# treangenlab/komb

Measured on NVIDIA B200. Metric: hot-path hits/s (graph build + k-core peel + CORE-A), with peel edges/s and build hits/s, higher is better.
Workload: dtype u32/u64 ids, f64 scores

## Files before the change

komb_b200/csrc/sort.cu:

```cuda
#include "kombgpu_debug.h"
#include "primitives.cuh"

namespace kg {

namespace {

constexpr int kRsThreads = 512;
constexpr int kRsItems = 8;
constexpr int kRsTile = kRsThreads * kRsItems;
constexpr int kRadix = 256;
constexpr int kMaxPasses = 8;

struct DigitSpec {
    int shift, shift2, bits1;
    uint32_t mask1, mask2, mask;
    __host__ __device__ static DigitSpec of(const RadixPass &p) {
        DigitSpec d;
        d.shift = p.shift; d.shift2 = p.shift2; d.bits1 = p.bits;
        d.mask1 = (1u << p.bits) - 1u; d.mask2 = (1u << p.bits2) - 1u;
        d.mask = (1u << (p.bits + p.bits2)) - 1u;
        return d;
    }
    __device__ __forceinline__ uint32_t operator()(uint64_t key) const {
        return ((uint32_t)(key >> shift) & mask1) | (((uint32_t)(key >> shift2) & mask2) << bits1);
    }
};


template <typename W>
struct StatusWord {
    static constexpr int kShift = 8 * (int)sizeof(W) - 2;
    static constexpr W kAgg = W(1) << kShift, kPrefix = W(2) << kShift, kValueMask = (W(1) << kShift) - 1;
    static __device__ __forceinline__ W load(const W *p) {
        W w;
        if constexpr (sizeof(W) == 4) asm volatile("ld.volatile.global.u32 %0, [%1];" : "=r"(w) : "l"(p) : "memory");
        else asm volatile("ld.volatile.global.u64 %0, [%1];" : "=l"(w) : "l"(p) : "memory");
        return w;
    }
    static __device__ __forceinline__ void store(W *p, W w) {
        if constexpr (sizeof(W) == 4) asm volatile("st.volatile.global.u32 [%0], %1;" ::"l"(p), "r"(w) : "memory");
        else asm volatile("st.volatile.global.u64 [%0], %1;" ::"l"(p), "l"(w) : "memory");
    }
};

struct PassList {
    DigitSpec dg[kMaxPasses];
    int n;
};

__global__ void __launch_bounds__(kRsThreads) radix_global_hist_kernel(const uint64_t *__restrict__ keys, uint64_t n, PassList pl,
                                                                       uint32_t *__restrict__ hist) {
    __shared__ uint32_t s_hist[kMaxPasses * kRadix];
    for (int i = threadIdx.x; i < pl.n * kRadix; i += kRsThreads) s_hist[i] = 0;
    __syncthreads();
    const uint32_t lane = lane_id();
    for (uint64_t base = (uint64_t)blockIdx.x * kRsTile; base < n; base += (uint64_t)gridDim.x * kRsTile) {
        uint64_t key[kRsItems];
#pragma unroll
        for (int j = 0; j < kRsItems; ++j) {
            const uint64_t i = base + (uint64_t)j * kRsThreads + threadIdx.x;
            key[j] = i < n ? keys[i] : ~0ull;
        }
#pragma unroll
        for (int j = 0; j < kRsItems; ++j) {
            const uint64_t i = base + (uint64_t)j * kRsThreads + threadIdx.x;
            const bool valid = i < n;
            const bool full = __all_sync(kFullMask, valid);
            for (int p = 0; p < pl.n; ++p) {
                const uint32_t d = pl.dg[p](key[j]);
                const uint32_t d0 = __shfl_sync(kFullMask, d, 0);
                if (full && __all_sync(kFullMask, d == d0)) {
                    if (lane == 0) atomicAdd(&s_hist[p * kRadix + d0], 32u);
                } else if (valid) {
                    atomicAdd(&s_hist[p * kRadix + d], 1u);
                }
            }
        }
    }
    __syncthreads();
    for (int i = threadIdx.x; i < pl.n * kRadix; i += kRsThreads)
        if (s_hist[i]) atomicAdd(&hist[i], s_hist[i]);
}

__global__ void __launch_bounds__(kRadix) radix_hist_scan_kernel(uint32_t *hist) {
    __shared__ uint32_t s_tmp[kRadix / 32 + 1];
    uint32_t *h = hist + (size_t)blockIdx.x * kRadix;
    const uint32_t v = h[threadIdx.x];
    uint32_t total = 0;
    const uint32_t ex = block_excl_scan_add<uint32_t, kRadix>(v, s_tmp, &total);
    h[threadIdx.x] = ex;
}

constexpr int kSweepThreads = 512, kSweepItems = 16, kSweepTile = kSweepThreads * kSweepItems, kSweepMinBlocks = 2;

struct SweepSmem {
    uint64_t keys[kSweepTile];
    uint32_t warp_cnt[kSweepThreads / 32][kRadix];
    uint32_t digit_local[kRadix];
    uint32_t digit_global[kRadix];
    uint32_t digit_total[kRadix];
    uint32_t tile;
};

template <typename W, int kBits>
__global__ void __launch_bounds__(kSweepThreads, kSweepMinBlocks) radix_sweep_kernel(const uint64_t *__restrict__ in, uint64_t *__restrict__ out,
                                                                    uint64_t n, DigitSpec dg,
                                                                    const uint32_t *__restrict__ digit_base,
                                                                    W *status, uint32_t *tile_counter) {
    using SW = StatusWord<W>;
    constexpr int kWarps = kSweepThreads / 32;
    extern __shared__ __align__(16) unsigned char s_raw[];
    SweepSmem &s = *reinterpret_cast<SweepSmem *>(s_raw);
    const uint32_t warp = threadIdx.x >> 5, lane = lane_id();
    const uint32_t mask = kBits ? (1u << kBits) - 1u : dg.mask;
    if (threadIdx.x == 0) s.tile = atomicAdd(tile_counter, 1u);
    for (int i = threadIdx.x; i < kWarps * kRadix; i += kSweepThreads) (&s.warp_cnt[0][0])[i] = 0;
    __syncthreads();
    const uint32_t tile = s.tile;
    const uint64_t tile_base = (uint64_t)tile * kSweepTile;
    const uint32_t tile_count = (uint32_t)min((uint64_t)kSweepTile, n - tile_base);

    uint64_t key[kSweepItems];
    uint16_t rank[kSweepItems];
    const uint32_t warp_base = warp * (32 * kSweepItems);
#pragma unroll
    for (int j = 0; j < kSweepItems; ++j) {
        const uint32_t e = warp_base + j * 32 + lane;
        key[j] = e < tile_count ? in[tile_base + e] : 0;
    }
#pragma unroll
    for (int j = 0; j < kSweepItems; ++j) {
        const uint32_t e = warp_base + j * 32 + lane;
        const bool valid = e < tile_count;
        const uint32_t d = valid ? dg(key[j]) : 0u;
        uint32_t same = __ballot_sync(kFullMask, valid);
#pragma unroll
        for (int b = 0; b < 8; ++b) {
            if (kBits ? (b >= kBits) : ((mask >> b) == 0)) break;
            const uint32_t bit = (d >> b) & 1u;
            const uint32_t vote = __ballot_sync(kFullMask, bit);
            same &= vote ^ (bit - 1u);
        }
        const uint32_t lead = valid ? (uint32_t)__ffs(same) - 1u : lane;
        uint32_t base = 0;
        if (valid && lead == lane) base = atomicAdd(&s.warp_cnt[warp][d], (uint32_t)__popc(same));
        rank[j] = (uint16_t)(__popc(same & lanemask_lt()) + __shfl_sync(kFullMask, base, lead));
    }
    __syncthreads();

    for (uint32_t d = threadIdx.x; d < (uint32_t)kRadix; d += kSweepThreads) {
        uint32_t total = 0;
#pragma unroll
        for (int w = 0; w < kWarps; ++w) {
            const uint32_t c = s.warp_cnt[w][d];
            s.warp_cnt[w][d] = total;
            total += c;
        }
        s.digit_total[d] = total;
        if (d <= mask) SW::store(status + (size_t)tile * kRadix + d, (tile == 0 ? SW::kPrefix : SW::kAgg) | (W)total);
    }
    __syncthreads();
    if (warp == 0) {
        uint32_t v[kRadix / 32], sum = 0;
#pragma unroll
        for (int i = 0; i < kRadix / 32; ++i) { v[i] = s.digit_total[lane * (kRadix / 32) + i]; sum += v[i]; }
        uint32_t run = warp_incl_scan_add(sum) - sum;
#pragma unroll
        for (int i = 0; i < kRadix / 32; ++i) { s.digit_local[lane * (kRadix / 32) + i] = run; run += v[i]; }
    }
    __syncthreads();

#pragma unroll
    for (int j = 0; j < kSweepItems; ++j) {
        const uint32_t e = warp_base + j * 32 + lane;
        if (e < tile_count) {
            const uint32_t d = dg(key[j]);
            s.keys[s.digit_local[d] + s.warp_cnt[warp][d] + rank[j]] = key[j];
        }
    }
    for (uint32_t d = threadIdx.x; d <= mask; d += kSweepThreads) {
        uint32_t excl = 0;
        if (tile > 0) {
            uint32_t p = tile - 1;
            uint32_t spins = 0;
            while (true) {
                const W w = SW::load(status + (size_t)p * kRadix + d);
                if ((w >> SW::kShift) == 0) {
                    if (++spins > (1u << 28)) __trap();
                    continue;
                }
                excl += (uint32_t)(w & SW::kValueMask);
                if (w & SW::kPrefix) break;
                --p;
            }
            SW::store(status + (size_t)tile * kRadix + d, SW::kPrefix | (W)(excl + s.digit_total[d]));
        }
        s.digit_global[d] = digit_base[d] + excl - s.digit_local[d];
    }
    __syncthreads();

    for (uint32_t i = threadIdx.x; i < tile_count; i += kSweepThreads) {
        const uint64_t k = s.keys[i];
        const uint32_t d = dg(k);
        out[(uint64_t)(s.digit_global[d] + i)] = k;
    }
}

template <typename W>
int sweep_pass(kombgpu_ctx *ctx, const uint64_t *src, uint64_t *dst, uint64_t n, const RadixPass &pass, const DigitSpec &dg,
               const uint32_t *digit_base, W *status, uint32_t *tile_counter) {
    auto *kernel = pass.bits + pass.bits2 == 8 ? radix_sweep_kernel<W, 8> : radix_sweep_kernel<W, 0>;
    KG_LAUNCH(ctx, kernel, ceil_div_u64(n, kSweepTile), kSweepThreads, sizeof(SweepSmem), src, dst, n, dg, digit_base, status,
              tile_counter);
    return KOMBGPU_OK;
}

}

int plan_radix_passes(int lo0, int hi0, int lo1, int hi1, RadixPass *out) {
    const int len0 = hi0 > lo0 ? hi0 - lo0 : 0, len1 = hi1 > lo1 ? hi1 - lo1 : 0;
    const int total = len0 + len1;
    if (total <= 0) return 0;
    const int np = (total + 7) / 8;
    const int w = (total + np - 1) / np;
    int n = 0;
    for (int v = 0; v < total; v += w) {
        const int e = v + w < total ? v + w : total;
        RadixPass p{0, 0, 0, 0};
        if (e <= len0) { p.shift = lo0 + v; p.bits = e - v; }
        else if (v >= len0) { p.shift = lo1 + (v - len0); p.bits = e - v; }
        else { p.shift = lo0 + v; p.bits = len0 - v; p.shift2 = lo1; p.bits2 = e - len0; }
        out[n++] = p;
    }
    return n;
}

int radix_sort_u64(kombgpu_ctx *ctx, uint64_t *a, uint64_t *b, uint64_t n, const RadixPass *passes, int n_passes,
                   uint64_t **sorted) {
    *sorted = a;
    if (n < 2 || n_passes == 0) return KOMBGPU_OK;
    if (n >= (1ull << 32)) return ctx_fail(ctx, KOMBGPU_EINVAL, "radix_sort_u64: %llu keys exceed the 2^32 per-array limit", (unsigned long long)n);
    if (n_passes > kMaxPasses) return ctx_fail(ctx, KOMBGPU_EINVAL, "radix_sort_u64: %d passes exceed %d", n_passes, kMaxPasses);
    if (!ctx->sort_attr_set) {
        KG_CUDA(ctx, cudaFuncSetAttribute(radix_sweep_kernel<uint32_t, 8>, cudaFuncAttributeMaxDynamicSharedMemorySize, (int)sizeof(SweepSmem)));
        KG_CUDA(ctx, cudaFuncSetAttribute(radix_sweep_kernel<uint32_t, 0>, cudaFuncAttributeMaxDynamicSharedMemorySize, (int)sizeof(SweepSmem)));
        KG_CUDA(ctx, cudaFuncSetAttribute(radix_sweep_kernel<uint64_t, 8>, cudaFuncAttributeMaxDynamicSharedMemorySize, (int)sizeof(SweepSmem)));
        KG_CUDA(ctx, cudaFuncSetAttribute(radix_sweep_kernel<uint64_t, 0>, cudaFuncAttributeMaxDynamicSharedMemorySize, (int)sizeof(SweepSmem)));
        ctx->sort_attr_set = true;
    }
    const bool wide = n >= (1ull << 30);
    const size_t region = (size_t)ceil_div_u64(n, kSweepTile) * kRadix;
    const size_t head = (size_t)n_passes * kRadix + kMaxPasses;
    const size_t words = head + (wide ? 2 * region : (size_t)n_passes * region);
    DevBuf<uint32_t> ws;
    KG_ALLOC(ctx, ws, words);
    KG_CUDA(ctx, cudaMemsetAsync(ws.p, 0, words * sizeof(uint32_t), ctx->stream));
    PassList pl{};
    pl.n = n_passes;
    for (int p = 0; p < n_passes; ++p) pl.dg[p] = DigitSpec::of(passes[p]);
    uint64_t *src = a, *dst = b;
    const uint32_t hist_grid = min(ceil_div_u64(n, kRsTile), (uint32_t)ctx->sm_count * 4u);
    KG_LAUNCH(ctx, radix_global_hist_kernel, hist_grid, kRsThreads, 0, src, n, pl, ws.p);
    KG_LAUNCH(ctx, radix_hist_scan_kernel, n_passes, kRadix, 0, ws.p);
    for (int p = 0; p < n_passes; ++p) {
        const uint32_t *digit_base = ws.p + (size_t)p * kRadix;
        uint32_t *counter = ws.p + (size_t)n_passes * kRadix + p;
        if (wide) {
            uint64_t *status = reinterpret_cast<uint64_t *>(ws.p + head);
            if (p > 0) KG_CUDA(ctx, cudaMemsetAsync(status, 0, region * sizeof(uint64_t), ctx->stream));
            KG_TRY(sweep_pass(ctx, src, dst, n, passes[p], pl.dg[p], digit_base, status, counter));
        } else {
            KG_TRY(sweep_pass(ctx, src, dst, n, passes[p], pl.dg[p], digit_base, ws.p + head + (size_t)p * region, counter));
        }
        uint64_t *t = src; src = dst; dst = t;
    }
    *sorted = src;
    return KOMBGPU_OK;
}


namespace {

__device__ __forceinline__ uint64_t mix64(uint64_t x) {
    x ^= x >> 33; x *= 0xff51afd7ed558ccdull; x ^= x >> 33; x *= 0xc4ceb9fe1a85ec53ull; x ^= x >> 33;
    return x;
}
__global__ void debug_fill_kernel(uint64_t *keys, uint64_t n, uint64_t lo_mask, uint64_t hi_mask, int sorted_hi) {
    for (uint64_t i = (uint64_t)blockIdx.x * blockDim.x + threadIdx.x; i < n; i += (uint64_t)gridDim.x * blockDim.x) {
        const uint64_t h = mix64(i + 0x9e3779b97f4a7c15ull);
        const uint64_t hi = sorted_hi ? ((i * (hi_mask + 1)) / n) : ((h >> 32) & hi_mask);
        keys[i] = (hi << 32) | (h & lo_mask);
    }
}
__global__ void debug_check_kernel(const uint64_t *keys, uint64_t n, unsigned long long *out) {
    unsigned long long sum = 0, x = 0, bad = 0;
    for (uint64_t i = (uint64_t)blockIdx.x * blockDim.x + threadIdx.x; i < n; i += (uint64_t)gridDim.x * blockDim.x) {
        sum += keys[i];
        x ^= mix64(keys[i]);
        if (i && keys[i - 1] > keys[i]) ++bad;
    }
    atomicAdd(&out[0], sum);
    atomicXor(&out[1], x);
    if (bad) atomicAdd(&out[2], bad);
}

}

}

extern "C" int kombgpu_debug_sort_u64(kombgpu_ctx *ctx, uint64_t n, int lo_bits, int hi_bits, int sorted_hi, int reps,
                                      float *ms_best, int *ok) {
    using namespace kg;
    if (!ctx || !ms_best || !ok || n == 0 || lo_bits < 0 || lo_bits > 32 || hi_bits < 0 || hi_bits > 32 || reps < 1)
        return KOMBGPU_EINVAL;
    KG_CUDA(ctx, cudaSetDevice(ctx->device));
    DevBuf<uint64_t> src, a, b;
    DevBuf<unsigned long long> chk;
    KG_ALLOC(ctx, src, n);
    KG_ALLOC(ctx, a, n);
    KG_ALLOC(ctx, b, n);
    KG_ALLOC(ctx, chk, 6);
    KG_CUDA(ctx, cudaMemsetAsync(chk.p, 0, 6 * sizeof(unsigned long long), ctx->stream));
    const uint64_t lo_mask = lo_bits == 32 ? 0xffffffffull : ((1ull << lo_bits) - 1), hi_mask = hi_bits == 32 ? 0xffffffffull : ((1ull << hi_bits) - 1);
    const int grid = ctx->sm_count * 8;
    KG_LAUNCH(ctx, debug_fill_kernel, grid, 256, 0, src.p, n, lo_mask, hi_mask, sorted_hi);
    KG_LAUNCH(ctx, debug_check_kernel, grid, 256, 0, src.p, n, chk.p);
    RadixPass passes[8];
    const int np = plan_radix_passes(0, lo_bits, 32, 32 + hi_bits, passes);
    float best = 1e30f;
    uint64_t *sorted = nullptr;
    cudaEvent_t e0, e1;
    KG_CUDA(ctx, cudaEventCreate(&e0));
    KG_CUDA(ctx, cudaEventCreate(&e1));
    for (int r = 0; r < reps; ++r) {
        KG_CUDA(ctx, cudaMemcpyAsync(a.p, src.p, n * sizeof(uint64_t), cudaMemcpyDeviceToDevice, ctx->stream));
        KG_CUDA(ctx, cudaEventRecord(e0, ctx->stream));
        int rc = radix_sort_u64(ctx, a.p, b.p, n, passes, np, &sorted);
        if (rc != KOMBGPU_OK) return rc;
        KG_CUDA(ctx, cudaEventRecord(e1, ctx->stream));
        KG_CUDA(ctx, cudaEventSynchronize(e1));
        float ms = 0;
        KG_CUDA(ctx, cudaEventElapsedTime(&ms, e0, e1));
        if (ms < best) best = ms;
    }
    cudaEventDestroy(e0);
    cudaEventDestroy(e1);
    KG_LAUNCH(ctx, debug_check_kernel, grid, 256, 0, sorted, n, chk.p + 3);
    unsigned long long h[6];
    KG_TRY(read_back(ctx, chk.p, h, 6));
    *ok = (h[0] == h[3] && h[1] == h[4] && h[5] == 0) ? 1 : 0;
    *ms_best = best;
    return KOMBGPU_OK;
}
```

Measured before the change: 2.840 billion.

## Widen onesweep radix digits to 10 bits with shared-memory match ranking

Raises the radix from 8 to 10 bits per pass so fewer sweep passes are needed per sort. Warp ranking moves from per-bit ballots to a shared-memory atomicOr match table, with a fast path for warps where all lanes share one digit. Per-warp counts become 16-bit and are handled as digit pairs, and status words are read and written with vector loads and stores. The status buffer is reused across passes with a per-pass memset, and keys are re-read from global memory in the scatter phase to save registers. Risks include bigger shared memory per block lowering occupancy, more decoupled-lookback traffic per tile, and shared-memory atomic contention.

```diff
diff --git a/komb_b200/csrc/sort.cu b/komb_b200/csrc/sort.cu
--- a/komb_b200/csrc/sort.cu
+++ b/komb_b200/csrc/sort.cu
@@ -8,7 +8,8 @@
 constexpr int kRsThreads = 512;
 constexpr int kRsItems = 8;
 constexpr int kRsTile = kRsThreads * kRsItems;
-constexpr int kRadix = 256;
+constexpr int kRadixBits = 10;
+constexpr int kRadix = 1 << kRadixBits;
 constexpr int kMaxPasses = 8;
 
 struct DigitSpec {
@@ -31,15 +32,13 @@
 struct StatusWord {
     static constexpr int kShift = 8 * (int)sizeof(W) - 2;
     static constexpr W kAgg = W(1) << kShift, kPrefix = W(2) << kShift, kValueMask = (W(1) << kShift) - 1;
-    static __device__ __forceinline__ W load(const W *p) {
-        W w;
-        if constexpr (sizeof(W) == 4) asm volatile("ld.volatile.global.u32 %0, [%1];" : "=r"(w) : "l"(p) : "memory");
-        else asm volatile("ld.volatile.global.u64 %0, [%1];" : "=l"(w) : "l"(p) : "memory");
-        return w;
-    }
-    static __device__ __forceinline__ void store(W *p, W w) {
-        if constexpr (sizeof(W) == 4) asm volatile("st.volatile.global.u32 [%0], %1;" ::"l"(p), "r"(w) : "memory");
-        else asm volatile("st.volatile.global.u64 [%0], %1;" ::"l"(p), "l"(w) : "memory");
+    static __device__ __forceinline__ void load2(const W *p, W &a, W &b) {
+        if constexpr (sizeof(W) == 4) asm volatile("ld.volatile.global.v2.u32 {%0, %1}, [%2];" : "=r"(a), "=r"(b) : "l"(p) : "memory");
+        else asm volatile("ld.volatile.global.v2.u64 {%0, %1}, [%2];" : "=l"(a), "=l"(b) : "l"(p) : "memory");
+    }
+    static __device__ __forceinline__ void store2(W *p, W a, W b) {
+        if constexpr (sizeof(W) == 4) asm volatile("st.volatile.global.v2.u32 [%0], {%1, %2};" ::"l"(p), "r"(a), "r"(b) : "memory");
+        else asm volatile("st.volatile.global.v2.u64 [%0], {%1, %2};" ::"l"(p), "l"(a), "l"(b) : "memory");
     }
 };
 
@@ -92,81 +91,98 @@
 }
 
 constexpr int kSweepThreads = 512, kSweepItems = 16, kSweepTile = kSweepThreads * kSweepItems, kSweepMinBlocks = 2;
+constexpr int kSweepWarps = kSweepThreads / 32;
+static_assert(kRadix == 2 * kSweepThreads, "the per-digit phases give every thread the digit pair 2t, 2t+1");
 
 struct SweepSmem {
-    uint64_t keys[kSweepTile];
-    uint32_t warp_cnt[kSweepThreads / 32][kRadix];
+    union {
+        uint64_t keys[kSweepTile];
+        uint32_t match[kSweepWarps][kRadix];
+    };
+    uint16_t warp_cnt[kSweepWarps][kRadix];
     uint32_t digit_local[kRadix];
     uint32_t digit_global[kRadix];
-    uint32_t digit_total[kRadix];
+    uint32_t pair_total[kSweepThreads];
+    uint32_t scan_tmp[kSweepWarps + 1];
     uint32_t tile;
 };
-
-template <typename W, int kBits>
+static_assert(kSweepTile <= 65535, "warp_cnt holds tile positions in 16 bits");
+
+template <typename W>
 __global__ void __launch_bounds__(kSweepThreads, kSweepMinBlocks) radix_sweep_kernel(const uint64_t *__restrict__ in, uint64_t *__restrict__ out,
                                                                     uint64_t n, DigitSpec dg,
                                                                     const uint32_t *__restrict__ digit_base,
                                                                     W *status, uint32_t *tile_counter) {
     using SW = StatusWord<W>;
-    constexpr int kWarps = kSweepThreads / 32;
     extern __shared__ __align__(16) unsigned char s_raw[];
     SweepSmem &s = *reinterpret_cast<SweepSmem *>(s_raw);
     const uint32_t warp = threadIdx.x >> 5, lane = lane_id();
-    const uint32_t mask = kBits ? (1u << kBits) - 1u : dg.mask;
+    const uint32_t mask = dg.mask, radix = mask + 1u;
     if (threadIdx.x == 0) s.tile = atomicAdd(tile_counter, 1u);
-    for (int i = threadIdx.x; i < kWarps * kRadix; i += kSweepThreads) (&s.warp_cnt[0][0])[i] = 0;
+    {
+        uint4 *m = reinterpret_cast<uint4 *>(&s.match[0][0]), *c = reinterpret_cast<uint4 *>(&s.warp_cnt[0][0]);
+        for (int i = threadIdx.x; i < (int)(sizeof(s.match) / sizeof(uint4)); i += kSweepThreads) m[i] = make_uint4(0, 0, 0, 0);
+        for (int i = threadIdx.x; i < (int)(sizeof(s.warp_cnt) / sizeof(uint4)); i += kSweepThreads) c[i] = make_uint4(0, 0, 0, 0);
+    }
     __syncthreads();
     const uint32_t tile = s.tile;
     const uint64_t tile_base = (uint64_t)tile * kSweepTile;
     const uint32_t tile_count = (uint32_t)min((uint64_t)kSweepTile, n - tile_base);
 
     uint64_t key[kSweepItems];
-    uint16_t rank[kSweepItems];
+    uint32_t rank[kSweepItems / 2];
     const uint32_t warp_base = warp * (32 * kSweepItems);
 #pragma unroll
     for (int j = 0; j < kSweepItems; ++j) {
         const uint32_t e = warp_base + j * 32 + lane;
         key[j] = e < tile_count ? in[tile_base + e] : 0;
     }
+    uint16_t *cnt = s.warp_cnt[warp];
+    uint32_t *match = s.match[warp];
 #pragma unroll
     for (int j = 0; j < kSweepItems; ++j) {
         const uint32_t e = warp_base + j * 32 + lane;
         const bool valid = e < tile_count;
-        const uint32_t d = valid ? dg(key[j]) : 0u;
-        uint32_t same = __ballot_sync(kFullMask, valid);
-#pragma unroll
-        for (int b = 0; b < 8; ++b) {
-            if (kBits ? (b >= kBits) : ((mask >> b) == 0)) break;
-            const uint32_t bit = (d >> b) & 1u;
-            const uint32_t vote = __ballot_sync(kFullMask, bit);
-            same &= vote ^ (bit - 1u);
-        }
-        const uint32_t lead = valid ? (uint32_t)__ffs(same) - 1u : lane;
+        const uint32_t d = dg(key[j]);
+        const uint32_t d0 = __shfl_sync(kFullMask, d, 0);
+        const bool uniform = __all_sync(kFullMask, valid && d == d0);
+        if (valid && !uniform) atomicOr(&match[d], 1u << lane);
+        __syncwarp();
+        const uint32_t peers = uniform ? kFullMask : valid ? match[d] : 0u;
+        const uint32_t lead = (uint32_t)__ffs(peers) - 1u;
+        __syncwarp();
         uint32_t base = 0;
-        if (valid && lead == lane) base = atomicAdd(&s.warp_cnt[warp][d], (uint32_t)__popc(same));
-        rank[j] = (uint16_t)(__popc(same & lanemask_lt()) + __shfl_sync(kFullMask, base, lead));
-    }
-    __syncthreads();
-
-    for (uint32_t d = threadIdx.x; d < (uint32_t)kRadix; d += kSweepThreads) {
-        uint32_t total = 0;
-#pragma unroll
-        for (int w = 0; w < kWarps; ++w) {
-            const uint32_t c = s.warp_cnt[w][d];
-            s.warp_cnt[w][d] = total;
-            total += c;
-        }
-        s.digit_total[d] = total;
-        if (d <= mask) SW::store(status + (size_t)tile * kRadix + d, (tile == 0 ? SW::kPrefix : SW::kAgg) | (W)total);
-    }
-    __syncthreads();
-    if (warp == 0) {
-        uint32_t v[kRadix / 32], sum = 0;
-#pragma unroll
-        for (int i = 0; i < kRadix / 32; ++i) { v[i] = s.digit_total[lane * (kRadix / 32) + i]; sum += v[i]; }
-        uint32_t run = warp_incl_scan_add(sum) - sum;
-#pragma unroll
-        for (int i = 0; i < kRadix / 32; ++i) { s.digit_local[lane * (kRadix / 32) + i] = run; run += v[i]; }
+        if (lead == lane) {
+            base = cnt[d];
+            cnt[d] = (uint16_t)(base + __popc(peers));
+            if (!uniform) match[d] = 0u;
+        }
+        const uint32_t r = __shfl_sync(kFullMask, base, lead & 31u) + __popc(peers & lanemask_lt());
+        __syncwarp();
+        rank[j / 2] = j % 2 ? rank[j / 2] | r << 16 : r;
+    }
+    __syncthreads();
+
+    const uint32_t d2 = 2u * threadIdx.x;
+    const bool pass_digits = d2 <= mask;
+    uint32_t tot2 = 0;
+#pragma unroll 4
+    for (int w = 0; w < kSweepWarps; ++w) {
+        uint32_t *wc = reinterpret_cast<uint32_t *>(s.warp_cnt[w]) + threadIdx.x;
+        const uint32_t c = *wc;
+        *wc = tot2;
+        tot2 += c;
+    }
+    if (pass_digits) {
+        const W flag = tile == 0 ? SW::kPrefix : SW::kAgg;
+        SW::store2(status + (size_t)tile * radix + d2, flag | (W)(tot2 & 0xffffu), flag | (W)(tot2 >> 16));
+    }
+    s.pair_total[threadIdx.x] = tot2;
+    {
+        uint32_t tile_total;
+        const uint32_t local = block_excl_scan_add<uint32_t, kSweepThreads>((tot2 & 0xffffu) + (tot2 >> 16), s.scan_tmp, &tile_total);
+        s.digit_local[d2] = local;
+        s.digit_local[d2 + 1] = local + (tot2 & 0xffffu);
     }
     __syncthreads();
 
@@ -174,28 +190,35 @@
     for (int j = 0; j < kSweepItems; ++j) {
         const uint32_t e = warp_base + j * 32 + lane;
         if (e < tile_count) {
-            const uint32_t d = dg(key[j]);
-            s.keys[s.digit_local[d] + s.warp_cnt[warp][d] + rank[j]] = key[j];
-        }
-    }
-    for (uint32_t d = threadIdx.x; d <= mask; d += kSweepThreads) {
-        uint32_t excl = 0;
+            const uint64_t k = in[tile_base + e];
+            const uint32_t d = dg(k);
+            s.keys[s.digit_local[d] + cnt[d] + ((rank[j / 2] >> (16 * (j % 2))) & 0xffffu)] = k;
+        }
+    }
+    if (pass_digits) {
+        const uint32_t tot_lo = s.pair_total[threadIdx.x] & 0xffffu, tot_hi = s.pair_total[threadIdx.x] >> 16;
+        W *my_status = status + (size_t)tile * radix + d2;
+        uint32_t ex_lo = 0, ex_hi = 0;
         if (tile > 0) {
             uint32_t p = tile - 1;
             uint32_t spins = 0;
+            bool done_lo = false, done_hi = false;
             while (true) {
-                const W w = SW::load(status + (size_t)p * kRadix + d);
-                if ((w >> SW::kShift) == 0) {
+                W w_lo, w_hi;
+                SW::load2(status + (size_t)p * radix + d2, w_lo, w_hi);
+                if ((!done_lo && (w_lo >> SW::kShift) == 0) || (!done_hi && (w_hi >> SW::kShift) == 0)) {
                     if (++spins > (1u << 28)) __trap();
                     continue;
                 }
-                excl += (uint32_t)(w & SW::kValueMask);
-                if (w & SW::kPrefix) break;
+                if (!done_lo) { ex_lo += (uint32_t)(w_lo & SW::kValueMask); done_lo = (w_lo & SW::kPrefix) != 0; }
+                if (!done_hi) { ex_hi += (uint32_t)(w_hi & SW::kValueMask); done_hi = (w_hi & SW::kPrefix) != 0; }
+                if (done_lo && done_hi) break;
                 --p;
             }
-            SW::store(status + (size_t)tile * kRadix + d, SW::kPrefix | (W)(excl + s.digit_total[d]));
-        }
-        s.digit_global[d] = digit_base[d] + excl - s.digit_local[d];
+            SW::store2(my_status, SW::kPrefix | (W)(ex_lo + tot_lo), SW::kPrefix | (W)(ex_hi + tot_hi));
+        }
+        s.digit_global[d2] = digit_base[d2] + ex_lo - s.digit_local[d2];
+        s.digit_global[d2 + 1] = digit_base[d2 + 1] + ex_hi - s.digit_local[d2 + 1];
     }
     __syncthreads();
 
@@ -207,10 +230,11 @@
 }
 
 template <typename W>
-int sweep_pass(kombgpu_ctx *ctx, const uint64_t *src, uint64_t *dst, uint64_t n, const RadixPass &pass, const DigitSpec &dg,
+int sweep_pass(kombgpu_ctx *ctx, const uint64_t *src, uint64_t *dst, uint64_t n, const DigitSpec &dg,
                const uint32_t *digit_base, W *status, uint32_t *tile_counter) {
-    auto *kernel = pass.bits + pass.bits2 == 8 ? radix_sweep_kernel<W, 8> : radix_sweep_kernel<W, 0>;
-    KG_LAUNCH(ctx, kernel, ceil_div_u64(n, kSweepTile), kSweepThreads, sizeof(SweepSmem), src, dst, n, dg, digit_base, status,
+    const uint32_t tiles = ceil_div_u64(n, kSweepTile);
+    KG_CUDA(ctx, cudaMemsetAsync(status, 0, (size_t)tiles * (dg.mask + 1u) * sizeof(W), ctx->stream));
+    KG_LAUNCH(ctx, radix_sweep_kernel<W>, tiles, kSweepThreads, sizeof(SweepSmem), src, dst, n, dg, digit_base, status,
               tile_counter);
     return KOMBGPU_OK;
 }
@@ -221,7 +245,7 @@
     const int len0 = hi0 > lo0 ? hi0 - lo0 : 0, len1 = hi1 > lo1 ? hi1 - lo1 : 0;
     const int total = len0 + len1;
     if (total <= 0) return 0;
-    const int np = (total + 7) / 8;
+    const int np = (total + kRadixBits - 1) / kRadixBits;
     const int w = (total + np - 1) / np;
     int n = 0;
     for (int v = 0; v < total; v += w) {
@@ -242,22 +266,26 @@
     if (n >= (1ull << 32)) return ctx_fail(ctx, KOMBGPU_EINVAL, "radix_sort_u64: %llu keys exceed the 2^32 per-array limit", (unsigned long long)n);
     if (n_passes > kMaxPasses) return ctx_fail(ctx, KOMBGPU_EINVAL, "radix_sort_u64: %d passes exceed %d", n_passes, kMaxPasses);
     if (!ctx->sort_attr_set) {
-        KG_CUDA(ctx, cudaFuncSetAttribute(radix_sweep_kernel<uint32_t, 8>, cudaFuncAttributeMaxDynamicSharedMemorySize, (int)sizeof(SweepSmem)));
-        KG_CUDA(ctx, cudaFuncSetAttribute(radix_sweep_kernel<uint32_t, 0>, cudaFuncAttributeMaxDynamicSharedMemorySize, (int)sizeof(SweepSmem)));
-        KG_CUDA(ctx, cudaFuncSetAttribute(radix_sweep_kernel<uint64_t, 8>, cudaFuncAttributeMaxDynamicSharedMemorySize, (int)sizeof(SweepSmem)));
-        KG_CUDA(ctx, cudaFuncSetAttribute(radix_sweep_kernel<uint64_t, 0>, cudaFuncAttributeMaxDynamicSharedMemorySize, (int)sizeof(SweepSmem)));
+        KG_CUDA(ctx, cudaFuncSetAttribute(radix_sweep_kernel<uint32_t>, cudaFuncAttributeMaxDynamicSharedMemorySize, (int)sizeof(SweepSmem)));
+        KG_CUDA(ctx, cudaFuncSetAttribute(radix_sweep_kernel<uint64_t>, cudaFuncAttributeMaxDynamicSharedMemorySize, (int)sizeof(SweepSmem)));
         ctx->sort_attr_set = true;
     }
     const bool wide = n >= (1ull << 30);
-    const size_t region = (size_t)ceil_div_u64(n, kSweepTile) * kRadix;
-    const size_t head = (size_t)n_passes * kRadix + kMaxPasses;
-    const size_t words = head + (wide ? 2 * region : (size_t)n_passes * region);
+    PassList pl{};
+    pl.n = n_passes;
+    uint32_t widest = 0;
+    for (int p = 0; p < n_passes; ++p) {
+        pl.dg[p] = DigitSpec::of(passes[p]);
+        if (passes[p].bits < 0 || passes[p].bits2 < 0 || passes[p].bits + passes[p].bits2 < 1 || passes[p].bits + passes[p].bits2 > kRadixBits)
+            return ctx_fail(ctx, KOMBGPU_EINVAL, "radix_sort_u64: pass %d has %d digit bits (1..%d)", p, passes[p].bits + passes[p].bits2, kRadixBits);
+        widest = max(widest, pl.dg[p].mask + 1u);
+    }
+    const size_t region = (size_t)ceil_div_u64(n, kSweepTile) * widest;
+    const size_t head = ((size_t)n_passes * kRadix + kMaxPasses + 3) & ~(size_t)3;
+    const size_t words = head + (wide ? 2 : 1) * region;
     DevBuf<uint32_t> ws;
     KG_ALLOC(ctx, ws, words);
-    KG_CUDA(ctx, cudaMemsetAsync(ws.p, 0, words * sizeof(uint32_t), ctx->stream));
-    PassList pl{};
-    pl.n = n_passes;
-    for (int p = 0; p < n_passes; ++p) pl.dg[p] = DigitSpec::of(passes[p]);
+    KG_CUDA(ctx, cudaMemsetAsync(ws.p, 0, head * sizeof(uint32_t), ctx->stream));
     uint64_t *src = a, *dst = b;
     const uint32_t hist_grid = min(ceil_div_u64(n, kRsTile), (uint32_t)ctx->sm_count * 4u);
     KG_LAUNCH(ctx, radix_global_hist_kernel, hist_grid, kRsThreads, 0, src, n, pl, ws.p);
@@ -265,13 +293,8 @@
     for (int p = 0; p < n_passes; ++p) {
         const uint32_t *digit_base = ws.p + (size_t)p * kRadix;
         uint32_t *counter = ws.p + (size_t)n_passes * kRadix + p;
-        if (wide) {
-            uint64_t *status = reinterpret_cast<uint64_t *>(ws.p + head);
-            if (p > 0) KG_CUDA(ctx, cudaMemsetAsync(status, 0, region * sizeof(uint64_t), ctx->stream));
-            KG_TRY(sweep_pass(ctx, src, dst, n, passes[p], pl.dg[p], digit_base, status, counter));
-        } else {
-            KG_TRY(sweep_pass(ctx, src, dst, n, passes[p], pl.dg[p], digit_base, ws.p + head + (size_t)p * region, counter));
-        }
+        if (wide) KG_TRY(sweep_pass(ctx, src, dst, n, pl.dg[p], digit_base, reinterpret_cast<uint64_t *>(ws.p + head), counter));
+        else KG_TRY(sweep_pass(ctx, src, dst, n, pl.dg[p], digit_base, ws.p + head, counter));
         uint64_t *t = src; src = dst; dst = t;
     }
     *sorted = src;
@@ -289,7 +312,7 @@
     for (uint64_t i = (uint64_t)blockIdx.x * blockDim.x + threadIdx.x; i < n; i += (uint64_t)gridDim.x * blockDim.x) {
         const uint64_t h = mix64(i + 0x9e3779b97f4a7c15ull);
         const uint64_t hi = sorted_hi ? ((i * (hi_mask + 1)) / n) : ((h >> 32) & hi_mask);
-        keys[i] = (hi << 32) | (h & lo_mask);
+        keys[i] = (hi << 32) | (lo_mask ? (h & lo_mask) : i);
     }
 }
 __global__ void debug_check_kernel(const uint64_t *keys, uint64_t n, unsigned long long *out) {
```

New measurement: 2.843 billion, median of 6. Within noise of the previous version (+0.1%).
